# fernandezdaniel/MOBOCMF

Measured on AMD Instinct MI355X. Metric: ELBO steps/sec (MFDGP d=8 M=512 N=8192 S=8), higher is better.
Workload: dtype f64

## Files before the change

include/mobocmf_hip.h:

```cpp
#ifndef MOBOCMF_HIP_H
#define MOBOCMF_HIP_H

#include <stddef.h>
#include <stdint.h>

#ifdef __cplusplus
extern "C" {
#endif

typedef void* mobocmf_stream_t;

#define MOBOCMF_MAX_D 32
#define MOBOCMF_MAX_XDIV 48

enum {
    MOBOCMF_OK = 0,
    MOBOCMF_BAD_ARG = 1,
    MOBOCMF_WORKSPACE_TOO_SMALL = 2,
    MOBOCMF_HIP_ERROR = 3,
    MOBOCMF_NOT_PD = 4,
    MOBOCMF_BAD_ARCH = 5
};

typedef struct mobocmf_tuning {
    uint32_t struct_size;
    int32_t small_gemm_max;
    int32_t small_panel_max;
    int32_t tile_rows;
    int32_t pair_mode;
    int32_t mid_gemm_max;
    int32_t mid_gemm_waves;
    int32_t syrk_workgroups;
    int32_t sparse_backward;
    int32_t potrf_cols;
} mobocmf_tuning;
int mobocmf_tuning_init(mobocmf_tuning* t);

typedef struct {
    int32_t kind;
    int32_t d;
    int32_t M;
    int32_t xdiv;
    int64_t Np;
    int32_t branch;
    int32_t want_dx;
    double jitter;
    double min_var;
    int32_t phase;
    int32_t reserved;
// ... 363 lines not shown
```

mobocmf_amd/_lib.py:

```python
import ctypes
import os

_HERE = os.path.dirname(os.path.abspath(__file__))
LIB_PATH = os.environ.get("MOBOCMF_HIP_LIB") or os.path.join(_HERE, "csrc", "libmobocmf_hip.so")

OK, BAD_ARG, WORKSPACE_TOO_SMALL, HIP_ERROR, NOT_PD, BAD_ARCH = range(6)
_ERR = {1: "MOBOCMF_BAD_ARG", 2: "MOBOCMF_WORKSPACE_TOO_SMALL", 3: "MOBOCMF_HIP_ERROR", 4: "MOBOCMF_NOT_PD",
        5: "MOBOCMF_BAD_ARCH"}


class Tuning(ctypes.Structure):
    _fields_ = [("struct_size", ctypes.c_uint32), ("small_gemm_max", ctypes.c_int32), ("small_panel_max", ctypes.c_int32),
                ("tile_rows", ctypes.c_int32), ("pair_mode", ctypes.c_int32), ("mid_gemm_max", ctypes.c_int32),
                ("mid_gemm_waves", ctypes.c_int32), ("syrk_workgroups", ctypes.c_int32), ("sparse_backward", ctypes.c_int32),
                ("potrf_cols", ctypes.c_int32)]
    KNOBS = tuple(n for n, _ in _fields_[1:])

    def copy(self):
        t = Tuning()
        ctypes.memmove(ctypes.byref(t), ctypes.byref(self), ctypes.sizeof(Tuning))
        return t


PROBE_EVENTS = 11


class LayerDesc(ctypes.Structure):
    _fields_ = [("kind", ctypes.c_int32), ("d", ctypes.c_int32), ("M", ctypes.c_int32), ("xdiv", ctypes.c_int32),
                ("Np", ctypes.c_int64), ("branch", ctypes.c_int32), ("want_dx", ctypes.c_int32),
                ("jitter", ctypes.c_double), ("min_var", ctypes.c_double), ("phase", ctypes.c_int32),
                ("reserved", ctypes.c_int32), ("tuning", ctypes.POINTER(Tuning)), ("probe_events", ctypes.c_void_p)]
# ... 213 lines not shown
```

mobocmf_amd/csrc/api.hip:

```cpp
#include "common.h"

int launch_gram_fwd(const GramArgs& g, hipStream_t s);
int launch_gram_bwd(const GramArgs& g, bool want_dx, hipStream_t s);
void gram_grid(const GramArgs& g, dim3* grid);
int launch_sum_partials(const double* part, int64_t P, int64_t stride, double* out, int64_t len, double scale,
                        int accumulate, hipStream_t s);
int launch_potrf(double* A, int64_t ld, int Mp, int M, double* Dinv, double* Ld, int32_t* info, hipStream_t s);
int launch_trtri(const double* L, int64_t ld, int Mp, const double* Dinv, double* Linv, double* T, double* ws,
                 int64_t ws_elems, hipStream_t s);
int launch_pad_tril(const double* src, int64_t lds, int M, double* dst, int Mp, hipStream_t s);
int launch_pad_vec(const double* src, int64_t n, double* dst, int64_t np, hipStream_t s);
int launch_transpose(const double* in, int64_t ldi, double* out, int64_t ldo, int64_t rows, int64_t cols, hipStream_t s);
int launch_gemv_rows(const double* Mat, int64_t ld, const double* vec, double* out, int rows, int64_t cols, double scale,
                     int accumulate, hipStream_t s);
int launch_kl(const double* L, const double* LSp, const double* U, const double* a, int M, int Mp, double* kl,
              double* part, hipStream_t s);
int launch_moments_finish(const double* qpart, const double* mupart, const double* rpart, int nrb, int64_t Np, int64_t N,
                          const double* knn, int branch, double min_var, double* q, double* r, double* varraw,
                          double* mean, double* var, int32_t* zero_word, hipStream_t s);
int launch_moments_bwd_prep(const double* g_mean, const double* g_var, const double* knn, const double* q,
                            const double* varraw, int branch, double min_var, int64_t N, int64_t Np, double* gmu,
                            double* gv, double* gv2, double* cgv, int32_t* nclamped, int zeroed, int32_t* blkact, hipStream_t s);
int launch_reduce_slabs_sym(const double* slabs, int64_t slab_stride, int nslab, int nslab_diag, double* out, int Mp, const int32_t* flag,
                            const double* fallback, hipStream_t s);
// ... 29 lines not shown
int launch_gemv_rows_z(const double* Mat, int64_t ld, const double* vec, double* out, int rows, int64_t cols, double scale,
                       int accumulate, int nz, int64_t zs, hipStream_t s);
int launch_transpose_pad_z(const double* in, double* out, int Mp, const double* const* LS, const double* const* m, int M,
                           double* LSp, double* mp, int nz, int64_t zs, hipStream_t s);
int launch_transpose_gemv_z(const double* in, double* out, int Mp, const double* Mat, const double* vec, double* vout, int nz,
                            int64_t zs, hipStream_t s);
int launch_kl_z(const double* L, const double* LSp, const double* U, const double* a, int M, int Mp, double* const* kl,
                double* part, int nz, int64_t zs, hipStream_t s);
int launch_dutot_y_z(const double* G1, const double* G2, const double* Hc, const double* U, const double* da, const double* a,
                     const double* const* gkl, int Mp, double* dU, double* da_tot, double* Y, int nz, int64_t zs, hipStream_t s);
int launch_dl_from_t2_z(const double* T2, const double* L, const double* const* gkl, int M, int Mp, double* dL, int nz,
                        int64_t zs, hipStream_t s);
int launch_phi_z(const double* T3, int Mp, double* P, int nz, int64_t zs, hipStream_t s);
int launch_symmetrize_z(const double* S, int Mp, double* G, int nz, int64_t zs, hipStream_t s);

static const mobocmf_tuning kDefaultTuning = {(uint32_t)sizeof(mobocmf_tuning), 384, 512, 0, 0, 1024, 32, 0, 1, 0};
static thread_local const mobocmf_tuning* t_tuning = nullptr;
static thread_local void* const* t_probe = nullptr;
const mobocmf_tuning& tune() { return t_tuning ? *t_tuning : kDefaultTuning; }
bool tuning_ok(const mobocmf_tuning* t) {
    if (!t) return true;
    return t->struct_size == sizeof(mobocmf_tuning) && t->small_gemm_max >= 1 && t->small_gemm_max <= 512 &&
           t->small_panel_max >= 1 && t->small_panel_max <= 512 && (t->tile_rows == 0 || t->tile_rows == 64 || t->tile_rows == 128) &&
           t->pair_mode >= 0 && t->pair_mode <= 2 && t->mid_gemm_max >= 0 && t->mid_gemm_max <= 4096 &&
           (t->mid_gemm_waves == 4 || t->mid_gemm_waves == 8 || t->mid_gemm_waves == 32) &&
           (t->syrk_workgroups == 0 || (t->syrk_workgroups >= 16 && t->syrk_workgroups <= 4096)) &&
           (t->sparse_backward == 0 || t->sparse_backward == 1) && (t->potrf_cols == 0 || t->potrf_cols == 1 || t->potrf_cols == 4);
}
TuneScope::TuneScope(const mobocmf_tuning* t, void* const* probe) : prev_t(t_tuning), prev_p(t_probe) {
    t_tuning = t;
    t_probe = probe;
}
TuneScope::~TuneScope() {
    t_tuning = prev_t;
    t_probe = prev_p;
}
void probe_at(int i, hipStream_t s) {
    if (t_probe && i < MOBOCMF_PROBE_EVENTS && t_probe[i]) (void)hipEventRecord((hipEvent_t)t_probe[i], s);
}
static void set_pairing(GemmArgs& g) { g.pair_mode = tune().pair_mode; }
static int panel_tile_rows(int, int64_t) { return tune().tile_rows; }

#define TRY(x)              \
    do {                    \
// ... 1051 lines not shown
```

mobocmf_amd/csrc/common.h:

```cpp
#pragma once
#include <hip/hip_runtime.h>
#include <stdint.h>

#include "../../include/mobocmf_hip.h"

#define TILE 128
#define NB 64

static inline int64_t round_up(int64_t v, int64_t m) { return (v + m - 1) / m * m; }

#define HIP_TRY(expr)                                   \
    do {                                                \
        hipError_t _e = (expr);                         \
        if (_e != hipSuccess) return MOBOCMF_HIP_ERROR; \
    } while (0)

const mobocmf_tuning& tune();
bool tuning_ok(const mobocmf_tuning* t);
void probe_at(int i, hipStream_t s);
struct TuneScope {
    const mobocmf_tuning* prev_t;
    void* const* prev_p;
    explicit TuneScope(const mobocmf_tuning* t, void* const* probe = nullptr);
    ~TuneScope();
    TuneScope(const TuneScope&) = delete;
    TuneScope& operator=(const TuneScope&) = delete;
};

enum { TRI_NONE = 0, TRI_LOWER_A = 1, TRI_UPPER_A = 2, TRI_LOWER_B = 4, TRI_UPPER_B = 8 };
enum { EPI_STORE = 0, EPI_COLSTATS = 1, EPI_DA = 2 };

struct GemmArgs {
    const double* A;
    const double* B;
    double* C;
    int64_t lda, ldb, ldc;
    int Mr;
// ... 115 lines not shown
```

mobocmf_amd/csrc/elementwise.hip:

```cpp
#include "common.h"

#define LOG_2PI 1.8378770664093454835606594728112

__device__ __forceinline__ double wave_sum(double v) {
    v += __shfl_xor(v, 1);
    v += __shfl_xor(v, 2);
    v += __shfl_xor(v, 4);
    v += __shfl_xor(v, 8);
    v += __shfl_xor(v, 16);
    v += __shfl_xor(v, 32);
    return v;
}

__device__ __forceinline__ double block_sum(double v, double* sh) {
    v = wave_sum(v);
    const int lane = threadIdx.x & 63, wave = threadIdx.x >> 6;
    __syncthreads();
    if (lane == 0) sh[wave] = v;
    __syncthreads();
    double t = 0.0;
    if (threadIdx.x == 0)
        for (int w = 0; w < (int)(blockDim.x >> 6); ++w) t += sh[w];
    return t;
}
// ... 300 lines not shown
        if (threadIdx.x < 2) {
            const int64_t blk = (int64_t)blockIdx.x * 2 + threadIdx.x;
            if (blk * 128 < Np) blkact[blk] = any_w[2 * threadIdx.x] | any_w[2 * threadIdx.x + 1];
        }
    }
}
int launch_moments_bwd_prep(const double* g_mean, const double* g_var, const double* knn, const double* q,
                            const double* varraw, int branch, double min_var, int64_t N, int64_t Np, double* gmu,
                            double* gv, double* gv2, double* cgv, int32_t* nclamped, int zeroed, int32_t* blkact, hipStream_t s) {
    if (!zeroed && launch_zero32(nclamped, 1, s)) return MOBOCMF_HIP_ERROR;
    hipLaunchKernelGGL(moments_bwd_prep_kernel, GRID1(Np), 0, s, g_mean, g_var, knn, q, varraw, branch, min_var, N, Np,
                       gmu, gv, gv2, cgv, nclamped, blkact);
    return CHECK_LAUNCH();
}

__device__ __forceinline__ double slab_sum(const double* p, int64_t slab_stride, int ns) {
    double v = 0.0;
    int z = 0;
    for (; z + 8 <= ns; z += 8) {
        double t[8];
#pragma unroll
        for (int b = 0; b < 8; ++b) t[b] = p[(z + b) * slab_stride];
#pragma unroll
        for (int b = 0; b < 8; ++b) v += t[b];
    }
    for (; z < ns; ++z) v += p[z * slab_stride];
    return v;
}

__global__ void reduce_slabs_sym_kernel(const double* slabs, int64_t slab_stride, int nslab, int nslab_diag, double* out,
                                        int Mp, const int32_t* flag, const double* fallback) {
    int64_t idx = (int64_t)blockIdx.x * blockDim.x + threadIdx.x;
    if (idx >= (int64_t)Mp * Mp) return;
    int i = (int)(idx / Mp), j = (int)(idx % Mp);
    if (flag && *flag == 0) {
        out[idx] = fallback[idx];
        return;
    }
    if (j / TILE > i / TILE) return;
    const double* p = j > i ? slabs + (int64_t)j * Mp + i : slabs + (int64_t)i * Mp + j;
    const int ns = (i / TILE == j / TILE) ? nslab_diag : nslab;
    const double v = slab_sum(p, slab_stride, ns);
    out[idx] = v;
    if (j / TILE < i / TILE) out[(int64_t)j * Mp + i] = v;
}
__global__ void reduce_slabs_sym2_kernel(const double* slabs, const double* slabs2, int64_t slab_stride, int nslab,
                                         int nslab_diag, double* out, double* out2, int Mp, const int32_t* flag) {
    int64_t idx = (int64_t)blockIdx.x * blockDim.x + threadIdx.x;
    if (idx >= (int64_t)Mp * Mp) return;
    int i = (int)(idx / Mp), j = (int)(idx % Mp);
    if (j / TILE > i / TILE) return;
    const int64_t off = j > i ? (int64_t)j * Mp + i : (int64_t)i * Mp + j;
    const int ns = (i / TILE == j / TILE) ? nslab_diag : nslab;
    const double v = slab_sum(slabs + off, slab_stride, ns);
    double v2 = v;
    if (*flag != 0) v2 = slab_sum(slabs2 + off, slab_stride, ns);
    out[idx] = v;
    out2[idx] = v2;
    if (j / TILE < i / TILE) { out[(int64_t)j * Mp + i] = v; out2[(int64_t)j * Mp + i] = v2; }
}
int launch_reduce_slabs_sym2(const double* slabs, const double* slabs2, int64_t slab_stride, int nslab, int nslab_diag,
                             double* out, double* out2, int Mp, const int32_t* flag, hipStream_t s) {
    hipLaunchKernelGGL(reduce_slabs_sym2_kernel, GRID1((int64_t)Mp * Mp), 0, s, slabs, slabs2, slab_stride, nslab, nslab_diag,
                       out, out2, Mp, flag);
    return CHECK_LAUNCH();
}
int launch_reduce_slabs_sym(const double* slabs, int64_t slab_stride, int nslab, int nslab_diag, double* out, int Mp,
                            const int32_t* flag, const double* fallback, hipStream_t s) {
    hipLaunchKernelGGL(reduce_slabs_sym_kernel, GRID1((int64_t)Mp * Mp), 0, s, slabs, slab_stride, nslab, nslab_diag, out, Mp,
                       flag, fallback);
    return CHECK_LAUNCH();
}

__global__ void dutot_y_kernel(const double* G1, const double* G2, const double* Hc, const double* U, const double* da,
                               const double* a, ScalZ gklz, int Mp, double* dU, double* da_tot, double* Y, int64_t zs) {
    __shared__ double tl[32][33];
    const double* gkl = gklz.p[blockIdx.z];
    const double g = gkl ? gkl[0] : 0.0;
    const int64_t zo = blockIdx.z * zs;
    G1 += zo; G2 += zo; Hc += zo; U += zo; da += zo; a += zo; dU += zo; da_tot += zo; Y += zo;
    const int nt = Mp / 32, ti = blockIdx.x / nt, tj = blockIdx.x % nt;
    const int tx = threadIdx.x & 31, ty = threadIdx.x >> 5;
    if (tj <= ti) {
#pragma unroll
        for (int r = ty; r < 32; r += 8) tl[r][tx] = G1[(int64_t)(tj * 32 + r) * Mp + ti * 32 + tx];
// ... 1115 lines not shown
```

mobocmf_amd/csrc/gemm_f64.hip:

```cpp
#include "common.h"
#include <type_traits>
#include <atomic>

typedef double v4f64 __attribute__((ext_vector_type(4)));
typedef double v2f64 __attribute__((ext_vector_type(2)));

#define BM 128
#define BN 128
#define BK 16
#define KL_MAX 1024
#define TILE_ELEMS (BM * BK)

#ifndef GEMM_MI
#define GEMM_MI 16
#endif
#if GEMM_MI == 16
#define IMG_SWZ(row) ((((row) >> 1) & 1) | ((((row) >> 3) & 1) << 2))
#else
#define IMG_SWZ(row) ((((row) >> 1) & 1) << 2)
#endif


template <int CTRL>
__device__ __forceinline__ double dpp_mov(double v) {
// ... 51 lines not shown
#define STEP_STAMPS_DECL unsigned long long sst[10] = {0, 0, 0, 0, 0, 0, 0, 0, 0, 0};
#define STEP_STAMP(i) do { if (sbase >= 0) sst[sbase + (i)] = __builtin_amdgcn_s_memrealtime(); } while (0)
#define STEP_STAMPS_FLUSH                                                                                   \
    do {                                                                                                    \
        if (g_stamp_buf && threadIdx.x == 0)                                                                \
            for (int q = 0; q < 10; ++q) g_stamp_buf[(int64_t)blockIdx.x * 32 + 16 + q] = sst[q];           \
    } while (0)
#else
#define STAMP(i)
#define STAMP_ID()
#define STEP_STAMPS_DECL
#define STEP_STAMP(i)
#define STEP_STAMPS_FLUSH
#endif

template <bool B_T, bool TRI, int EPI, int RM>
__global__ __launch_bounds__(256, RM == 64 ? 3 : 2) void gemm_f64_kernel(GemmArgs g, int nrb, int64_t ncb, int splitk, int pair) {
    static_assert(RM == 128 || (RM == 64 && !B_T), "tile heights: 128, or 64 for the A B form");
    constexpr int MT = RM / 32;
    constexpr int A_ELEMS = RM * BK;
    constexpr int STAGE_ELEMS = A_ELEMS + TILE_ELEMS;
    __shared__ __attribute__((aligned(16))) double lds[2 * STAGE_ELEMS];
    __shared__ int kl[B_T ? KL_MAX : 1];
    __shared__ int kl_wsum[4];
    if (g.skip_if_zero && *g.skip_if_zero == 0) return;
    STAMP(0);
    STAMP_ID();
    int64_t id = blockIdx.x;
    if (g.dual_flag) {
        const int64_t half = (int64_t)(gridDim.x >> 1);
        if (id >= half) {
            if (*g.dual_flag == 0) return;
            id -= half;
            g.bscale = g.bscale2;
            g.C = g.C2;
        }
    }
    int rb, z = 0, sk_eff = splitk;
    int64_t cb;
    if (g.batched) {
        z = blockIdx.z;
        cb = id / nrb;
        rb = nrb - 1 - (int)(id % nrb);
    } else if (splitk > 1 && g.lower_out && g.splitk_diag > 0) {
        const int64_t nF = (int64_t)nrb * (nrb - 1) / 2, nblkF = nF * splitk;
        const bool diag = id >= nblkF;
        const int64_t id2 = diag ? id - nblkF : id, nT = diag ? nrb : nF;
        sk_eff = diag ? g.splitk_diag : splitk;
        int64_t t;
        if ((sk_eff & 7) == 0 && (nblkF & 7) == 0) {
            const int64_t xcd = id2 & 7, seq = id2 >> 3;
            t = seq % nT;
            z = (int)((seq / nT) * 8 + xcd);
        } else {
            t = id2 % nT;
            z = (int)(id2 / nT);
        }
        if (diag) {
            rb = (int)t;
            cb = t;
        } else {
            int r = 1;
            while ((int64_t)r * (r + 1) / 2 <= t) ++r;
            rb = r;
            cb = t - (int64_t)r * (r - 1) / 2;
        }
    } else if (splitk > 1) {
        const int64_t ntile = g.lower_out ? (int64_t)nrb * (nrb + 1) / 2 : (int64_t)nrb * ncb;
        int64_t t;
        if ((splitk & 7) == 0) {
            const int64_t xcd = id & 7, seq = id >> 3;
            t = seq % ntile;
            z = (int)((seq / ntile) * 8 + xcd);
        } else {
            t = id % ntile;
            z = (int)(id / ntile);
        }
        if (g.lower_out) {
            int r = 0;
            while ((int64_t)(r + 1) * (r + 2) / 2 <= t) ++r;
            rb = r;
            cb = t - (int64_t)r * (r + 1) / 2;
        } else {
            cb = t / nrb;
            rb = (int)(t % nrb);
        }
    } else {
        const int nslot = pair ? (nrb + 1) / 2 : nrb;
        int sl;
        if ((ncb & 7) == 0) {
            int64_t xcd = id & 7, slot = id >> 3;
            cb = (slot / nslot) * 8 + xcd;
            sl = (int)(slot % nslot);
        } else {
            cb = id / nslot;
            sl = (int)(id % nslot);
        }
        rb = pair ? sl : nrb - 1 - sl;
    }
    if (g.lower_out && cb > rb) return;

    const double* A = g.A;
    const double* B = g.B;
    double* C = g.C;
    if (g.batched) {
        const int zl = g.zlayers > 1 ? z % g.zlayers : 0;
        const int zb = g.zlayers > 1 ? z / g.zlayers : z;
        A += zb * g.strideA + zl * g.zsA;
        B += zb * g.strideB + zl * g.zsB;
        C += zb * g.strideC + zl * g.zsC;
    }
    if (!g.batched && splitk > 1) {
        C += z * g.slab_stride;
        if (g.zlayers > 1) {
            A += blockIdx.z * g.zsA;
            B += blockIdx.z * g.zsB;
            C += blockIdx.z * g.zsC;
        }
    }
    const int nparts = (pair && rb != nrb - 1 - rb) ? 2 : 1;
    const int rb_first = rb;

    const int tid = threadIdx.x;
    const int lane = tid & 63;
    const int wave = __builtin_amdgcn_readfirstlane(tid >> 6);
    const int wr = wave >> 1, wc = wave & 1;
    const int li = lane & 15, lk = lane >> 4;

    if constexpr (!B_T) {
        if (g.colact && g.colact[cb] == 0) {
            if (EPI == EPI_DA && g.rowdot_part) {
                for (int part = 0; part < nparts; ++part) {
                    const int rbp = part == 0 ? rb_first : nrb - 1 - rb_first;
                    for (int i = tid; i < 2 * RM; i += 256)
// ... 57 lines not shown
    if (g.tri & TRI_LOWER_B) {
        int64_t b = cb * BN;
        if (k0 < b) k0 = b;
    }
    if (g.tri & TRI_UPPER_B) {
        int64_t e = (cb + 1) * BN;
        if (k1 > e) k1 = e;
    }
    bool compact = false;
    int64_t ct0 = 0;
    int co0 = 0;
    if (!g.batched && splitk > 1) {
        bool sliced = false;
        if constexpr (B_T) {
            if (g.kact) {
                const int nb = (int)(g.Kd / 128), run = (nb + 255) / 256;
                const int rb0 = tid * run < nb ? tid * run : nb, rb1 = rb0 + run < nb ? rb0 + run : nb;
                int cnt = 0;
                for (int b = rb0; b < rb1; ++b) cnt += g.kact[b] != 0 ? 1 : 0;
                int inc = cnt;
#pragma unroll
                for (int off = 1; off < 64; off <<= 1) {
                    const int v = __shfl_up(inc, off);
                    if (lane >= off) inc += v;
                }
                if (lane == 63) kl_wsum[wave] = inc;
                __syncthreads();
                int ord = inc - cnt;
                for (int w = 0; w < wave; ++w) ord += kl_wsum[w];
                const int64_t nkt = (int64_t)(kl_wsum[0] + kl_wsum[1] + kl_wsum[2] + kl_wsum[3]) * (128 / BK);
                const int64_t per = (nkt + sk_eff - 1) / sk_eff;
                const int64_t tb = z * per < nkt ? z * per : nkt, te = tb + per < nkt ? tb + per : nkt;
                ct0 = tb;
                co0 = (int)(tb / (128 / BK));
                const int co1 = te > tb ? (int)((te - 1) / (128 / BK)) : co0 - 1;
                for (int b = rb0; b < rb1; ++b)
                    if (g.kact[b] != 0) {
                        if (ord >= co0 && ord <= co1 && ord - co0 < KL_MAX) kl[ord - co0] = b;
                        ++ord;
                    }
                __syncthreads();
                compact = true;
                sliced = true;
                k0 = 0;
                k1 = (te - tb) * BK;
            }
        }
        if (!sliced) {
            int64_t nkt = k1 > k0 ? (k1 - k0) / BK : 0;
            int64_t per = (nkt + sk_eff - 1) / sk_eff;
            int64_t b = k0 + z * per * BK, e = b + per * BK;
            k0 = b < k1 ? b : k1;
            k1 = e < k1 ? e : k1;
        }
    }
    const double* Ag = Ag0 + (int64_t)rb * RM * g.lda;

    v4f64 acc[MT][4];
#pragma unroll
    for (int i = 0; i < MT; ++i)
#pragma unroll
        for (int j = 0; j < 4; ++j) acc[i][j] = (v4f64){0.0, 0.0, 0.0, 0.0};

    const int64_t nk = (k1 > k0) ? (k1 - k0) / BK : 0;
#define KSTEP(KT) (rev ? nk - 1 - (KT) : (KT))
    auto koff = [&](int64_t kt) -> int64_t {
        if (B_T && compact) {
            const int64_t t = ct0 + kt;
            return (int64_t)kl[(int)(t / (128 / BK)) - co0] * 128 + (t % (128 / BK)) * BK;
        }
        return k0 + KSTEP(kt) * BK;
    };
#define KOFF(KT) koff(KT)
    if (nk > 0) stage(Ag, KOFF(0), 0);

    asm volatile("s_waitcnt vmcnt(0)" ::: "memory");
    __syncthreads();
    STAMP(1 + 4 * part);
    v4f64 w_nxt = (v4f64){1.0, 1.0, 1.0, 1.0};
    if (B_T && g.bscale && nk > 0) w_nxt = *(const v4f64*)(g.bscale + KOFF(0) + 4 * lk);
#if GEMM_MI == 16
    v2f64 fa[MT][2];
    double fb[4][4];
#define LOAD_A16(MT_)                                                                                       \
    fa[MT_][0] = *(const v2f64*)(As + a_base + (MT_) * 32 * BK + colP0);                                    \
// ... 359 lines not shown
    }
#define ST_PLAIN(v, p) (*(p) = (v))
#define ST_STREAM(v, p) __builtin_nontemporal_store((v), (p))
    if (g.accumulate) { STORE_TILE(ST_PLAIN, ST_PLAIN, 1) }
    else if (g.stream_out) { STORE_TILE(ST_STREAM, ST_STREAM, 0) }
    else { STORE_TILE(ST_PLAIN, ST_PLAIN, 0) }
#undef STORE_TILE
    if (part == 0) STAMP(13);

#undef COLOFF
    STAMP(9 + part);
  }
  STEP_STAMPS_FLUSH;
}

static bool small_panel_ok(const GemmArgs& g, bool B_T, int splitk);
template <int EPI> static int launch_small_panel(const GemmArgs& g, hipStream_t s);
static bool small_gemm_ok(const GemmArgs& g, bool B_T);
static int launch_small_gemm(const GemmArgs& g, bool B_T, hipStream_t s);

static int tile_rows(const GemmArgs& g, bool B_T, int splitk) {
    if (B_T || splitk > 1 || g.batched || g.lower_out || g.zlayers > 1) return BM;
    if (g.rm == 64 || g.rm == BM) return g.rm;
    if (!(g.tri & (TRI_LOWER_A | TRI_UPPER_A))) return BM;
    const int64_t pairs128 = (int64_t)((g.Mr / BM + 1) / 2) * (g.Nc / BN);
    return pairs128 >= 512 ? BM : 64;
}

int launch_gemm(const GemmArgs& g0, bool B_T, int splitk, hipStream_t s) {
    GemmArgs g = g0;
    if (g.Mr % BM || g.Nc % 16 || g.Kd % BK) return MOBOCMF_BAD_ARG;
    if (B_T || g.batched || splitk > 1) g.colact = nullptr;
    if (g.kact) {
        const int sk_min = (g.lower_out && g.splitk_diag > 0 && g.splitk_diag < splitk) ? g.splitk_diag : splitk;
        const int64_t nb = g.Kd / 128;
        if (!B_T || g.batched || splitk <= 1 || g.zlayers > 1 || g.Kd % 128 || (g.tri & (TRI_LOWER_B | TRI_UPPER_B)) ||
            (nb + sk_min - 1) / sk_min + 2 > KL_MAX)
            g.kact = nullptr;
    }
    if (!B_T && ((g.ldc & 1) || ((uintptr_t)g.C & 15))) return MOBOCMF_BAD_ARG;
    if (small_panel_ok(g, B_T, splitk)) {
// ... 29 lines not shown
    const bool tri = (g.tri & (TRI_LOWER_A | TRI_UPPER_A)) != 0 || g.epi == EPI_STORE;
#ifdef GEMM_LDS_PAD64
    const size_t dyn64 = GEMM_LDS_PAD64;
#define LAUNCH(BT, TR, EP, RM_)                                                                                         \
    do {                                                                                                                \
        const size_t dyn = (RM_) == 64 ? dyn64 : 0;                                                                     \
        if (dyn) (void)hipFuncSetAttribute((const void*)gemm_f64_kernel<BT, TR, EP, RM_>,                               \
                                           hipFuncAttributeMaxDynamicSharedMemorySize, (int)dyn);                       \
        hipLaunchKernelGGL((gemm_f64_kernel<BT, TR, EP, RM_>), grid, dim3(256), dyn, s, g, nrb, ncb, splitk, pair);      \
    } while (0)
#else
#define LAUNCH(BT, TR, EP, RM_) hipLaunchKernelGGL((gemm_f64_kernel<BT, TR, EP, RM_>), grid, dim3(256), 0, s, g, nrb, ncb, splitk, pair)
#endif
    if (B_T) {
        if (g.epi != EPI_STORE) return MOBOCMF_BAD_ARG;
        LAUNCH(true, false, EPI_STORE, 128);
    } else if (rm == 64) {
        if (g.epi == EPI_COLSTATS) LAUNCH(false, true, EPI_COLSTATS, 64);
        else if (g.epi == EPI_DA) LAUNCH(false, true, EPI_DA, 64);
        else LAUNCH(false, true, EPI_STORE, 64);
    } else if (tri) {
        if (g.epi == EPI_COLSTATS) LAUNCH(false, true, EPI_COLSTATS, 128);
        else if (g.epi == EPI_DA) LAUNCH(false, true, EPI_DA, 128);
        else LAUNCH(false, true, EPI_STORE, 128);
    } else {
        if (g.epi == EPI_COLSTATS) LAUNCH(false, false, EPI_COLSTATS, 128);
        else if (g.epi == EPI_DA) LAUNCH(false, false, EPI_DA, 128);
        else LAUNCH(false, false, EPI_STORE, 128);
    }
#undef LAUNCH
    return hipGetLastError() == hipSuccess ? MOBOCMF_OK : MOBOCMF_HIP_ERROR;
// ... 736 lines not shown
```

mobocmf_amd/functional.py:

```python
import contextlib
import ctypes
import os
import threading

import torch

from . import _lib
from ._lib import LayerDesc

JITTER = 1e-6
MIN_VARIANCE = 1e-10

_scratch = {}


def _stream():
    return ctypes.c_void_p(torch.cuda.current_stream().cuda_stream)


def _ptr(t):
    return ctypes.c_void_p(0 if t is None else t.data_ptr())


def _prep(t):
# ... 76 lines not shown
    if _TUNING_DEFAULT is None:
        t = _lib.Tuning()
        _lib.check(_lib.load().mobocmf_tuning_init(ctypes.byref(t)), "mobocmf_tuning_init")
        _TUNING_DEFAULT = t
    return _TUNING_DEFAULT


def current_tuning():
    t = getattr(_tuning_tls, "override", None)
    return (t if t is not None else _default_tuning()).copy()


def _set_default(**kw):
    t = _default_tuning()
    for k, v in kw.items():
        assert k in _lib.Tuning.KNOBS, k
        setattr(t, k, int(v))


@contextlib.contextmanager
def tuning(**kw):
    prev = getattr(_tuning_tls, "override", None)
    t = current_tuning()
    for k, v in kw.items():
        if k not in _lib.Tuning.KNOBS:
            raise TypeError("unknown tuning knob %r" % k)
        setattr(t, k, int(v))
    _tuning_tls.override = t
    try:
        yield t
    finally:
        _tuning_tls.override = prev


_probe_tls = threading.local()


@contextlib.contextmanager
def probe_events(table, layer=None):
    prev = getattr(_probe_tls, "cur", None)
# ... 1275 lines not shown
    _set_default(mid_gemm_max=n)


def set_mid_gemm_waves(n=32):
    if int(n) not in (4, 8, 32):
        raise _lib.MobocmfError("set_mid_gemm_waves: 4 | 8 | 32")
    _set_default(mid_gemm_waves=n)


def set_syrk_workgroups(n=0):
    if int(n) != 0 and not 16 <= int(n) <= 4096:
        raise _lib.MobocmfError("set_syrk_workgroups: 0 | 16..4096")
    _set_default(syrk_workgroups=n)


def set_sparse_backward(on=True):
    _set_default(sparse_backward=1 if on else 0)


_block_act_tls = threading.local()


def set_block_activity(act=None):
    if act is not None:
        assert act.dtype == torch.int32 and act.is_cuda and act.is_contiguous()
    _block_act_tls.act = act


def set_tile_rows(rows=0, pair_mode=0):
    if int(rows) not in (0, 64, 128) or not 0 <= int(pair_mode) <= 2:
# ... 559 lines not shown
```

Before: 1069.

## Add 8-wave SYRK kernel option and vectorize symmetric slab reduction

Adds a new 512-thread, 8-wave split-K SYRK kernel for symmetric lower-output GEMMs. It is selected only through a new syrk_waves tuning knob, which defaults to off, and the tuning struct gains a backward-compatible field. Separately, the symmetric slab-reduction kernels now load two doubles at a time and use larger unrolled batches. Each thread covers its own lower-triangle entries and mirrors them, replacing the old tile-granular mapping. These changes aim to cut the memory-bound reduction cost and, when the knob is set, the SYRK launch cost, at the price of extra code paths and alignment checks.

```diff
diff --git a/include/mobocmf_hip.h b/include/mobocmf_hip.h
--- a/include/mobocmf_hip.h
+++ b/include/mobocmf_hip.h
@@ -33,6 +33,7 @@
     int32_t syrk_workgroups;
     int32_t sparse_backward;
     int32_t potrf_cols;
+    int32_t syrk_waves;
 } mobocmf_tuning;
 int mobocmf_tuning_init(mobocmf_tuning* t);
 
diff --git a/mobocmf_amd/_lib.py b/mobocmf_amd/_lib.py
--- a/mobocmf_amd/_lib.py
+++ b/mobocmf_amd/_lib.py
@@ -13,8 +13,9 @@
     _fields_ = [("struct_size", ctypes.c_uint32), ("small_gemm_max", ctypes.c_int32), ("small_panel_max", ctypes.c_int32),
                 ("tile_rows", ctypes.c_int32), ("pair_mode", ctypes.c_int32), ("mid_gemm_max", ctypes.c_int32),
                 ("mid_gemm_waves", ctypes.c_int32), ("syrk_workgroups", ctypes.c_int32), ("sparse_backward", ctypes.c_int32),
-                ("potrf_cols", ctypes.c_int32)]
-    KNOBS = tuple(n for n, _ in _fields_[1:])
+                ("potrf_cols", ctypes.c_int32), ("syrk_waves", ctypes.c_int32)]
+    KNOBS = tuple(n for n, _ in _fields_[1:10])
+    ALL_KNOBS = tuple(n for n, _ in _fields_[1:])
 
     def copy(self):
         t = Tuning()
diff --git a/mobocmf_amd/csrc/api.hip b/mobocmf_amd/csrc/api.hip
--- a/mobocmf_amd/csrc/api.hip
+++ b/mobocmf_amd/csrc/api.hip
@@ -1,3 +1,5 @@
+#include <string.h>
+#include <stddef.h>
 #include "common.h"
 
 int launch_gram_fwd(const GramArgs& g, hipStream_t s);
@@ -67,20 +69,34 @@
 int launch_phi_z(const double* T3, int Mp, double* P, int nz, int64_t zs, hipStream_t s);
 int launch_symmetrize_z(const double* S, int Mp, double* G, int nz, int64_t zs, hipStream_t s);
 
-static const mobocmf_tuning kDefaultTuning = {(uint32_t)sizeof(mobocmf_tuning), 384, 512, 0, 0, 1024, 32, 0, 1, 0};
+static const mobocmf_tuning kDefaultTuning = {(uint32_t)sizeof(mobocmf_tuning), 384, 512, 0, 0, 1024, 32, 0, 1, 0, 0};
+static const uint32_t kTuningSizeV1 = (uint32_t)offsetof(mobocmf_tuning, syrk_waves);
 static thread_local const mobocmf_tuning* t_tuning = nullptr;
 static thread_local void* const* t_probe = nullptr;
 const mobocmf_tuning& tune() { return t_tuning ? *t_tuning : kDefaultTuning; }
 bool tuning_ok(const mobocmf_tuning* t) {
     if (!t) return true;
+    if (t->struct_size == kTuningSizeV1) {
+        mobocmf_tuning full = kDefaultTuning;
+        memcpy(&full, t, kTuningSizeV1);
+        full.struct_size = (uint32_t)sizeof(mobocmf_tuning);
+        return tuning_ok(&full);
+    }
     return t->struct_size == sizeof(mobocmf_tuning) && t->small_gemm_max >= 1 && t->small_gemm_max <= 512 &&
            t->small_panel_max >= 1 && t->small_panel_max <= 512 && (t->tile_rows == 0 || t->tile_rows == 64 || t->tile_rows == 128) &&
            t->pair_mode >= 0 && t->pair_mode <= 2 && t->mid_gemm_max >= 0 && t->mid_gemm_max <= 4096 &&
            (t->mid_gemm_waves == 4 || t->mid_gemm_waves == 8 || t->mid_gemm_waves == 32) &&
            (t->syrk_workgroups == 0 || (t->syrk_workgroups >= 16 && t->syrk_workgroups <= 4096)) &&
-           (t->sparse_backward == 0 || t->sparse_backward == 1) && (t->potrf_cols == 0 || t->potrf_cols == 1 || t->potrf_cols == 4);
+           (t->sparse_backward == 0 || t->sparse_backward == 1) && (t->potrf_cols == 0 || t->potrf_cols == 1 || t->potrf_cols == 4) &&
+           (t->syrk_waves == 0 || t->syrk_waves == 4 || t->syrk_waves == 8);
 }
 TuneScope::TuneScope(const mobocmf_tuning* t, void* const* probe) : prev_t(t_tuning), prev_p(t_probe) {
+    if (t && t->struct_size == kTuningSizeV1) {
+        widened = kDefaultTuning;
+        memcpy(&widened, t, kTuningSizeV1);
+        widened.struct_size = (uint32_t)sizeof(mobocmf_tuning);
+        t = &widened;
+    }
     t_tuning = t;
     t_probe = probe;
 }
diff --git a/mobocmf_amd/csrc/common.h b/mobocmf_amd/csrc/common.h
--- a/mobocmf_amd/csrc/common.h
+++ b/mobocmf_amd/csrc/common.h
@@ -21,6 +21,7 @@
 struct TuneScope {
     const mobocmf_tuning* prev_t;
     void* const* prev_p;
+    mobocmf_tuning widened;
     explicit TuneScope(const mobocmf_tuning* t, void* const* probe = nullptr);
     ~TuneScope();
     TuneScope(const TuneScope&) = delete;
diff --git a/mobocmf_amd/csrc/elementwise.hip b/mobocmf_amd/csrc/elementwise.hip
--- a/mobocmf_amd/csrc/elementwise.hip
+++ b/mobocmf_amd/csrc/elementwise.hip
@@ -338,61 +338,121 @@
     return CHECK_LAUNCH();
 }
 
-__device__ __forceinline__ double slab_sum(const double* p, int64_t slab_stride, int ns) {
-    double v = 0.0;
+typedef double slab_v2 __attribute__((ext_vector_type(2)));
+template <int BATCH, bool FULL, typename T, typename LD>
+__device__ __forceinline__ void slab_batch(T& v, const LD& ld, int z, int ns) {
+    T t[BATCH];
+#pragma unroll
+    for (int b = 0; b < BATCH; ++b) t[b] = ld(FULL || z + b < ns ? z + b : ns - 1);
+#pragma unroll
+    for (int b = 0; b < BATCH; ++b)
+        if (FULL || z + b < ns) v += t[b];
+}
+template <typename T, typename LD>
+__device__ __forceinline__ T slab_sum(const LD& ld, int ns) {
+    T v = {};
     int z = 0;
-    for (; z + 8 <= ns; z += 8) {
-        double t[8];
-#pragma unroll
-        for (int b = 0; b < 8; ++b) t[b] = p[(z + b) * slab_stride];
-#pragma unroll
-        for (int b = 0; b < 8; ++b) v += t[b];
-    }
-    for (; z < ns; ++z) v += p[z * slab_stride];
+    for (; z + 32 <= ns; z += 32) slab_batch<32, true>(v, ld, z, ns);
+    const int rem = ns - z;
+    if (rem > 16) slab_batch<32, false>(v, ld, z, ns);
+    else if (rem > 8) slab_batch<16, false>(v, ld, z, ns);
+    else if (rem > 0) slab_batch<8, false>(v, ld, z, ns);
     return v;
 }
-
-__global__ void reduce_slabs_sym_kernel(const double* slabs, int64_t slab_stride, int nslab, int nslab_diag, double* out,
-                                        int Mp, const int32_t* flag, const double* fallback) {
-    int64_t idx = (int64_t)blockIdx.x * blockDim.x + threadIdx.x;
+__device__ __forceinline__ slab_v2 slab_sum_v2(const double* p0, int64_t slab_stride, int ns) {
+    const slab_v2* p = (const slab_v2*)p0;
+    const int64_t st = slab_stride >> 1;
+    return slab_sum<slab_v2>([=](int z) { return p[z * st]; }, ns);
+}
+__device__ __forceinline__ double slab_sum_one(const double* p, int64_t slab_stride, int ns) {
+    return slab_sum<double>([=](int z) { return p[z * slab_stride]; }, ns);
+}
+
+template <int W>
+__global__ __launch_bounds__(256) void reduce_slabs_sym_kernel(const double* slabs, int64_t slab_stride, int nslab, int nslab_diag,
+                                                               double* out, int Mp, const int32_t* flag, const double* fallback) {
+    const int64_t idx = ((int64_t)blockIdx.x * blockDim.x + threadIdx.x) * W;
     if (idx >= (int64_t)Mp * Mp) return;
-    int i = (int)(idx / Mp), j = (int)(idx % Mp);
+    const int i = (int)(idx / Mp), j = (int)(idx % Mp);
     if (flag && *flag == 0) {
-        out[idx] = fallback[idx];
+        if (W == 2) *(slab_v2*)(out + idx) = *(const slab_v2*)(fallback + idx);
+        else out[idx] = fallback[idx];
         return;
     }
-    if (j / TILE > i / TILE) return;
-    const double* p = j > i ? slabs + (int64_t)j * Mp + i : slabs + (int64_t)i * Mp + j;
+    if (j > i) return;
     const int ns = (i / TILE == j / TILE) ? nslab_diag : nslab;
-    const double v = slab_sum(p, slab_stride, ns);
-    out[idx] = v;
-    if (j / TILE < i / TILE) out[(int64_t)j * Mp + i] = v;
-}
-__global__ void reduce_slabs_sym2_kernel(const double* slabs, const double* slabs2, int64_t slab_stride, int nslab,
-                                         int nslab_diag, double* out, double* out2, int Mp, const int32_t* flag) {
-    int64_t idx = (int64_t)blockIdx.x * blockDim.x + threadIdx.x;
+    if (W == 2) {
+        const slab_v2 v = slab_sum_v2(slabs + idx, slab_stride, ns);
+        if (j == i) {
+            out[idx] = v[0];
+        } else {
+            *(slab_v2*)(out + idx) = v;
+            out[(int64_t)j * Mp + i] = v[0];
+            if (j + 1 < i) out[(int64_t)(j + 1) * Mp + i] = v[1];
+        }
+    } else {
+        const double v = slab_sum_one(slabs + idx, slab_stride, ns);
+        out[idx] = v;
+        if (j < i) out[(int64_t)j * Mp + i] = v;
+    }
+}
+template <int W>
+__global__ __launch_bounds__(256) void reduce_slabs_sym2_kernel(const double* slabs, const double* slabs2, int64_t slab_stride,
+                                                                int nslab, int nslab_diag, double* out, double* out2, int Mp,
+                                                                const int32_t* flag) {
+    const int64_t idx = ((int64_t)blockIdx.x * blockDim.x + threadIdx.x) * W;
     if (idx >= (int64_t)Mp * Mp) return;
-    int i = (int)(idx / Mp), j = (int)(idx % Mp);
-    if (j / TILE > i / TILE) return;
-    const int64_t off = j > i ? (int64_t)j * Mp + i : (int64_t)i * Mp + j;
+    const int i = (int)(idx / Mp), j = (int)(idx % Mp);
+    if (j > i) return;
     const int ns = (i / TILE == j / TILE) ? nslab_diag : nslab;
-    const double v = slab_sum(slabs + off, slab_stride, ns);
-    double v2 = v;
-    if (*flag != 0) v2 = slab_sum(slabs2 + off, slab_stride, ns);
-    out[idx] = v;
-    out2[idx] = v2;
-    if (j / TILE < i / TILE) { out[(int64_t)j * Mp + i] = v; out2[(int64_t)j * Mp + i] = v2; }
+    const bool twin = *flag != 0;
+    if (W == 2) {
+        const slab_v2 v = slab_sum_v2(slabs + idx, slab_stride, ns);
+        slab_v2 v2 = v;
+        if (twin) v2 = slab_sum_v2(slabs2 + idx, slab_stride, ns);
+        if (j == i) {
+            out[idx] = v[0];
+            out2[idx] = v2[0];
+        } else {
+            *(slab_v2*)(out + idx) = v;
+            *(slab_v2*)(out2 + idx) = v2;
+            out[(int64_t)j * Mp + i] = v[0];
+            out2[(int64_t)j * Mp + i] = v2[0];
+            if (j + 1 < i) {
+                out[(int64_t)(j + 1) * Mp + i] = v[1];
+                out2[(int64_t)(j + 1) * Mp + i] = v2[1];
+            }
+        }
+    } else {
+        const double v = slab_sum_one(slabs + idx, slab_stride, ns);
+        double v2 = v;
+        if (twin) v2 = slab_sum_one(slabs2 + idx, slab_stride, ns);
+        out[idx] = v;
+        out2[idx] = v2;
+        if (j < i) { out[(int64_t)j * Mp + i] = v; out2[(int64_t)j * Mp + i] = v2; }
+    }
+}
+static bool aligned16(const void* a, const void* b, const void* c, const void* d) {
+    return ((((uintptr_t)a) | ((uintptr_t)b) | ((uintptr_t)c) | ((uintptr_t)d)) & 15) == 0;
 }
 int launch_reduce_slabs_sym2(const double* slabs, const double* slabs2, int64_t slab_stride, int nslab, int nslab_diag,
                              double* out, double* out2, int Mp, const int32_t* flag, hipStream_t s) {
-    hipLaunchKernelGGL(reduce_slabs_sym2_kernel, GRID1((int64_t)Mp * Mp), 0, s, slabs, slabs2, slab_stride, nslab, nslab_diag,
-                       out, out2, Mp, flag);
+    if (aligned16(slabs, slabs2, out, out2) && !(slab_stride & 1))
+        hipLaunchKernelGGL(reduce_slabs_sym2_kernel<2>, GRID1((int64_t)Mp * Mp / 2), 0, s, slabs, slabs2, slab_stride, nslab,
+                           nslab_diag, out, out2, Mp, flag);
+    else
+        hipLaunchKernelGGL(reduce_slabs_sym2_kernel<1>, GRID1((int64_t)Mp * Mp), 0, s, slabs, slabs2, slab_stride, nslab,
+                           nslab_diag, out, out2, Mp, flag);
     return CHECK_LAUNCH();
 }
 int launch_reduce_slabs_sym(const double* slabs, int64_t slab_stride, int nslab, int nslab_diag, double* out, int Mp,
                             const int32_t* flag, const double* fallback, hipStream_t s) {
-    hipLaunchKernelGGL(reduce_slabs_sym_kernel, GRID1((int64_t)Mp * Mp), 0, s, slabs, slab_stride, nslab, nslab_diag, out, Mp,
-                       flag, fallback);
+    if (aligned16(slabs, out, fallback, nullptr) && !(slab_stride & 1))
+        hipLaunchKernelGGL(reduce_slabs_sym_kernel<2>, GRID1((int64_t)Mp * Mp / 2), 0, s, slabs, slab_stride, nslab, nslab_diag,
+                           out, Mp, flag, fallback);
+    else
+        hipLaunchKernelGGL(reduce_slabs_sym_kernel<1>, GRID1((int64_t)Mp * Mp), 0, s, slabs, slab_stride, nslab, nslab_diag, out,
+                           Mp, flag, fallback);
     return CHECK_LAUNCH();
 }
 
diff --git a/mobocmf_amd/csrc/gemm_f64.hip b/mobocmf_amd/csrc/gemm_f64.hip
--- a/mobocmf_amd/csrc/gemm_f64.hip
+++ b/mobocmf_amd/csrc/gemm_f64.hip
@@ -89,23 +89,20 @@
 #define STEP_STAMPS_FLUSH
 #endif
 
-template <bool B_T, bool TRI, int EPI, int RM>
-__global__ __launch_bounds__(256, RM == 64 ? 3 : 2) void gemm_f64_kernel(GemmArgs g, int nrb, int64_t ncb, int splitk, int pair) {
-    static_assert(RM == 128 || (RM == 64 && !B_T), "tile heights: 128, or 64 for the A B form");
-    constexpr int MT = RM / 32;
-    constexpr int A_ELEMS = RM * BK;
-    constexpr int STAGE_ELEMS = A_ELEMS + TILE_ELEMS;
-    __shared__ __attribute__((aligned(16))) double lds[2 * STAGE_ELEMS];
-    __shared__ int kl[B_T ? KL_MAX : 1];
-    __shared__ int kl_wsum[4];
-    if (g.skip_if_zero && *g.skip_if_zero == 0) return;
-    STAMP(0);
-    STAMP_ID();
+struct TileId {
+    int rb;
+    int64_t cb;
+    int z;
+    int sk_eff;
+};
+
+__device__ __forceinline__ bool gemm_tile_of_block(GemmArgs& g, int nrb, int64_t ncb, int splitk, int pair, TileId& t) {
+    if (g.skip_if_zero && *g.skip_if_zero == 0) return false;
     int64_t id = blockIdx.x;
     if (g.dual_flag) {
         const int64_t half = (int64_t)(gridDim.x >> 1);
         if (id >= half) {
-            if (*g.dual_flag == 0) return;
+            if (*g.dual_flag == 0) return false;
             id -= half;
             g.bscale = g.bscale2;
             g.C = g.C2;
@@ -122,43 +119,43 @@
         const bool diag = id >= nblkF;
         const int64_t id2 = diag ? id - nblkF : id, nT = diag ? nrb : nF;
         sk_eff = diag ? g.splitk_diag : splitk;
-        int64_t t;
+        int64_t tl;
         if ((sk_eff & 7) == 0 && (nblkF & 7) == 0) {
             const int64_t xcd = id2 & 7, seq = id2 >> 3;
-            t = seq % nT;
+            tl = seq % nT;
             z = (int)((seq / nT) * 8 + xcd);
         } else {
-            t = id2 % nT;
+            tl = id2 % nT;
             z = (int)(id2 / nT);
         }
         if (diag) {
-            rb = (int)t;
-            cb = t;
+            rb = (int)tl;
+            cb = tl;
         } else {
             int r = 1;
-            while ((int64_t)r * (r + 1) / 2 <= t) ++r;
+            while ((int64_t)r * (r + 1) / 2 <= tl) ++r;
             rb = r;
-            cb = t - (int64_t)r * (r - 1) / 2;
+            cb = tl - (int64_t)r * (r - 1) / 2;
         }
     } else if (splitk > 1) {
         const int64_t ntile = g.lower_out ? (int64_t)nrb * (nrb + 1) / 2 : (int64_t)nrb * ncb;
-        int64_t t;
+        int64_t tl;
         if ((splitk & 7) == 0) {
             const int64_t xcd = id & 7, seq = id >> 3;
-            t = seq % ntile;
+            tl = seq % ntile;
             z = (int)((seq / ntile) * 8 + xcd);
         } else {
-            t = id % ntile;
+            tl = id % ntile;
             z = (int)(id / ntile);
         }
         if (g.lower_out) {
             int r = 0;
-            while ((int64_t)(r + 1) * (r + 2) / 2 <= t) ++r;
+            while ((int64_t)(r + 1) * (r + 2) / 2 <= tl) ++r;
             rb = r;
-            cb = t - (int64_t)r * (r + 1) / 2;
+            cb = tl - (int64_t)r * (r + 1) / 2;
         } else {
-            cb = t / nrb;
-            rb = (int)(t % nrb);
+            cb = tl / nrb;
+            rb = (int)(tl % nrb);
         }
     } else {
         const int nslot = pair ? (nrb + 1) / 2 : nrb;
@@ -173,11 +170,19 @@
         }
         rb = pair ? sl : nrb - 1 - sl;
     }
-    if (g.lower_out && cb > rb) return;
-
-    const double* A = g.A;
-    const double* B = g.B;
-    double* C = g.C;
+    if (g.lower_out && cb > rb) return false;
+    t.rb = rb;
+    t.cb = cb;
+    t.z = z;
+    t.sk_eff = sk_eff;
+    return true;
+}
+
+__device__ __forceinline__ void gemm_operand_bases(const GemmArgs& g, int z, int splitk, const double*& A, const double*& B,
+                                                   double*& C) {
+    A = g.A;
+    B = g.B;
+    C = g.C;
     if (g.batched) {
         const int zl = g.zlayers > 1 ? z % g.zlayers : 0;
         const int zb = g.zlayers > 1 ? z / g.zlayers : z;
@@ -193,6 +198,73 @@
             C += blockIdx.z * g.zsC;
         }
     }
+}
+
+template <int NT>
+__device__ __forceinline__ int64_t kact_slice(const GemmArgs& g, int z, int sk_eff, int* kl, int* kl_wsum, int tid, int lane,
+                                              int wave, int64_t& ct0, int& co0) {
+    const int nb = (int)(g.Kd / 128), run = (nb + NT - 1) / NT;
+    const int rb0 = tid * run < nb ? tid * run : nb, rb1 = rb0 + run < nb ? rb0 + run : nb;
+    int cnt = 0;
+    for (int b = rb0; b < rb1; ++b) cnt += g.kact[b] != 0 ? 1 : 0;
+    int inc = cnt;
+#pragma unroll
+    for (int off = 1; off < 64; off <<= 1) {
+        const int v = __shfl_up(inc, off);
+        if (lane >= off) inc += v;
+    }
+    if (lane == 63) kl_wsum[wave] = inc;
+    __syncthreads();
+    int ord = inc - cnt, nact = 0;
+    for (int w = 0; w < wave; ++w) ord += kl_wsum[w];
+#pragma unroll
+    for (int w = 0; w < NT / 64; ++w) nact += kl_wsum[w];
+    const int64_t nkt = (int64_t)nact * (128 / BK);
+    const int64_t per = (nkt + sk_eff - 1) / sk_eff;
+    const int64_t tb = z * per < nkt ? z * per : nkt, te = tb + per < nkt ? tb + per : nkt;
+    ct0 = tb;
+    co0 = (int)(tb / (128 / BK));
+    const int co1 = te > tb ? (int)((te - 1) / (128 / BK)) : co0 - 1;
+    for (int b = rb0; b < rb1; ++b)
+        if (g.kact[b] != 0) {
+            if (ord >= co0 && ord <= co1 && ord - co0 < KL_MAX) kl[ord - co0] = b;
+            ++ord;
+        }
+    __syncthreads();
+    return te - tb;
+}
+__device__ __forceinline__ int64_t kact_koff(const int* kl, int64_t ct0, int co0, int64_t kt) {
+    const int64_t t = ct0 + kt;
+    return (int64_t)kl[(int)(t / (128 / BK)) - co0] * 128 + (t % (128 / BK)) * BK;
+}
+__device__ __forceinline__ void k_slice(int64_t& k0, int64_t& k1, int z, int sk_eff) {
+    const int64_t nkt = k1 > k0 ? (k1 - k0) / BK : 0;
+    const int64_t per = (nkt + sk_eff - 1) / sk_eff;
+    const int64_t b = k0 + z * per * BK, e = b + per * BK;
+    k0 = b < k1 ? b : k1;
+    k1 = e < k1 ? e : k1;
+}
+
+template <bool B_T, bool TRI, int EPI, int RM>
+__global__ __launch_bounds__(256, RM == 64 ? 3 : 2) void gemm_f64_kernel(GemmArgs g, int nrb, int64_t ncb, int splitk, int pair) {
+    static_assert(RM == 128 || (RM == 64 && !B_T), "tile heights: 128, or 64 for the A B form");
+    constexpr int MT = RM / 32;
+    constexpr int A_ELEMS = RM * BK;
+    constexpr int STAGE_ELEMS = A_ELEMS + TILE_ELEMS;
+    __shared__ __attribute__((aligned(16))) double lds[2 * STAGE_ELEMS];
+    __shared__ int kl[B_T ? KL_MAX : 1];
+    __shared__ int kl_wsum[4];
+    TileId tile;
+    if (!gemm_tile_of_block(g, nrb, ncb, splitk, pair, tile)) return;
+    STAMP(0);
+    STAMP_ID();
+    int rb = tile.rb;
+    const int z = tile.z, sk_eff = tile.sk_eff;
+    const int64_t cb = tile.cb;
+
+    const double *A, *B;
+    double* C;
+    gemm_operand_bases(g, z, splitk, A, B, C);
     const int nparts = (pair && rb != nrb - 1 - rb) ? 2 : 1;
     const int rb_first = rb;
 
@@ -280,45 +352,14 @@
         bool sliced = false;
         if constexpr (B_T) {
             if (g.kact) {
-                const int nb = (int)(g.Kd / 128), run = (nb + 255) / 256;
-                const int rb0 = tid * run < nb ? tid * run : nb, rb1 = rb0 + run < nb ? rb0 + run : nb;
-                int cnt = 0;
-                for (int b = rb0; b < rb1; ++b) cnt += g.kact[b] != 0 ? 1 : 0;
-                int inc = cnt;
-#pragma unroll
-                for (int off = 1; off < 64; off <<= 1) {
-                    const int v = __shfl_up(inc, off);
-                    if (lane >= off) inc += v;
-                }
-                if (lane == 63) kl_wsum[wave] = inc;
-                __syncthreads();
-                int ord = inc - cnt;
-                for (int w = 0; w < wave; ++w) ord += kl_wsum[w];
-                const int64_t nkt = (int64_t)(kl_wsum[0] + kl_wsum[1] + kl_wsum[2] + kl_wsum[3]) * (128 / BK);
-                const int64_t per = (nkt + sk_eff - 1) / sk_eff;
-                const int64_t tb = z * per < nkt ? z * per : nkt, te = tb + per < nkt ? tb + per : nkt;
-                ct0 = tb;
-                co0 = (int)(tb / (128 / BK));
-                const int co1 = te > tb ? (int)((te - 1) / (128 / BK)) : co0 - 1;
-                for (int b = rb0; b < rb1; ++b)
-                    if (g.kact[b] != 0) {
-                        if (ord >= co0 && ord <= co1 && ord - co0 < KL_MAX) kl[ord - co0] = b;
-                        ++ord;
-                    }
-                __syncthreads();
+                const int64_t nsteps = kact_slice<256>(g, z, sk_eff, kl, kl_wsum, tid, lane, wave, ct0, co0);
                 compact = true;
                 sliced = true;
                 k0 = 0;
-                k1 = (te - tb) * BK;
+                k1 = nsteps * BK;
             }
         }
-        if (!sliced) {
-            int64_t nkt = k1 > k0 ? (k1 - k0) / BK : 0;
-            int64_t per = (nkt + sk_eff - 1) / sk_eff;
-            int64_t b = k0 + z * per * BK, e = b + per * BK;
-            k0 = b < k1 ? b : k1;
-            k1 = e < k1 ? e : k1;
-        }
+        if (!sliced) k_slice(k0, k1, z, sk_eff);
     }
     const double* Ag = Ag0 + (int64_t)rb * RM * g.lda;
 
@@ -331,10 +372,7 @@
     const int64_t nk = (k1 > k0) ? (k1 - k0) / BK : 0;
 #define KSTEP(KT) (rev ? nk - 1 - (KT) : (KT))
     auto koff = [&](int64_t kt) -> int64_t {
-        if (B_T && compact) {
-            const int64_t t = ct0 + kt;
-            return (int64_t)kl[(int)(t / (128 / BK)) - co0] * 128 + (t % (128 / BK)) * BK;
-        }
+        if (B_T && compact) return kact_koff(kl, ct0, co0, kt);
         return k0 + KSTEP(kt) * BK;
     };
 #define KOFF(KT) koff(KT)
@@ -724,6 +762,151 @@
   STEP_STAMPS_FLUSH;
 }
 
+#if GEMM_MI == 16
+#define W8_LE0 0xD5
+#define W8_LE1 0xF4
+#define W8_LT0 0x54
+#define W8_LT1 0xD0
+__global__ __launch_bounds__(512) void syrk_w8_kernel(GemmArgs g, int nrb, int64_t ncb, int splitk) {
+    constexpr int STAGE_ELEMS = 2 * TILE_ELEMS;
+    __shared__ __attribute__((aligned(16))) double lds[2 * STAGE_ELEMS];
+    __shared__ int kl[KL_MAX];
+    __shared__ int kl_wsum[8];
+    TileId tile;
+    if (!gemm_tile_of_block(g, nrb, ncb, splitk, 0, tile)) return;
+    const int rb = tile.rb, z = tile.z;
+    const int64_t cb = tile.cb;
+    const double *A, *B;
+    double* C;
+    gemm_operand_bases(g, z, splitk, A, B, C);
+
+    const int tid = threadIdx.x;
+    const int lane = tid & 63;
+    const int wave = __builtin_amdgcn_readfirstlane(tid >> 6);
+    const int wr = (wave >> 1) & 1, wc = wave & 1, h = wave >> 2;
+    const int li = lane & 15, lk = lane >> 4;
+
+    const int a_row = tid >> 3;
+    const int a_lchk = (tid & 7) ^ IMG_SWZ(a_row);
+    const double* Ag = A + ((int64_t)rb * BM + a_row) * g.lda + a_lchk * 2;
+    const double* Bg = B + (cb * BN + a_row) * g.ldb + a_lchk * 2;
+    auto stage = [&](int64_t k, int buf) {
+        double* As = lds + buf * STAGE_ELEMS;
+        double* Bs = As + TILE_ELEMS;
+#pragma unroll
+        for (int r = 0; r < 2; ++r) glds16(Ag + (int64_t)(64 * r) * g.lda + k, As + (r * 8 + wave) * 128);
+#pragma unroll
+        for (int r = 0; r < 2; ++r) glds16(Bg + (int64_t)(64 * r) * g.ldb + k, Bs + (r * 8 + wave) * 128);
+    };
+
+    int64_t k0 = 0, k1 = g.Kd, ct0 = 0;
+    int co0 = 0;
+    const bool compact = g.kact != nullptr;
+    if (compact) {
+        k1 = kact_slice<512>(g, z, tile.sk_eff, kl, kl_wsum, tid, lane, wave, ct0, co0) * BK;
+    } else {
+        k_slice(k0, k1, z, tile.sk_eff);
+    }
+    const int64_t nk = (k1 > k0) ? (k1 - k0) / BK : 0;
+    auto koff = [&](int64_t kt) -> int64_t { return compact ? kact_koff(kl, ct0, co0, kt) : k0 + kt * BK; };
+
+    const int swA = IMG_SWZ(li);
+    const int colP0 = ((2 * lk + 0) ^ swA) << 1, colP1 = ((2 * lk + 1) ^ swA) << 1;
+    const int a_base = (wr * 16 + li) * BK;
+    const int b_base0 = ((h ? 1 : 0) * 32 + wc * 16 + li) * BK;
+    const int b_base1 = ((h ? 2 : 3) * 32 + wc * 16 + li) * BK;
+
+    v4f64 acc[4][2];
+#pragma unroll
+    for (int i = 0; i < 4; ++i)
+#pragma unroll
+        for (int j = 0; j < 2; ++j) acc[i][j] = (v4f64){0.0, 0.0, 0.0, 0.0};
+
+    if (nk > 0) stage(koff(0), 0);
+    asm volatile("s_waitcnt vmcnt(0)" ::: "memory");
+    __syncthreads();
+    v4f64 w_nxt = (v4f64){1.0, 1.0, 1.0, 1.0};
+    if (g.bscale && nk > 0) w_nxt = *(const v4f64*)(g.bscale + koff(0) + 4 * lk);
+#ifdef SYRK_W8_PRIO
+    if (h) __builtin_amdgcn_s_setprio(1);
+#endif
+
+    v2f64 fa[4][2];
+    double fb[4][2];
+#define W8_ROW(MASK, MT_) ((((MASK) >> (2 * (MT_))) & 3) != 0)
+#define W8_COL(MASK, J) ((((MASK) >> (J)) & 0x55) != 0)
+#define W8_LOAD_A(MASK, MT_, CH)                                                                            \
+    if constexpr (W8_ROW(MASK, MT_)) fa[MT_][CH] = *(const v2f64*)(As + a_base + (MT_) * 32 * BK + ((CH) ? colP1 : colP0));
+#define W8_LOAD_B(MASK, J, CH)                                                                              \
+    if constexpr (W8_COL(MASK, J)) {                                                                        \
+        const v2f64 v = *(const v2f64*)(Bs + ((J) ? b_base1 : b_base0) + ((CH) ? colP1 : colP0));           \
+        fb[2 * (CH)][J] = v[0] * w4[2 * (CH)];                                                              \
+        fb[2 * (CH) + 1][J] = v[1] * w4[2 * (CH) + 1];                                                      \
+    }
+#define W8_MMA(MASK, Q, MT_, J)                                                                             \
+    if constexpr ((((MASK) >> (2 * (MT_) + (J))) & 1) != 0)                                                 \
+        acc[MT_][J] = __builtin_amdgcn_mfma_f64_16x16x4f64(fa[MT_][(Q) >> 1][(Q) & 1], fb[Q][J], acc[MT_][J], 0, 0, 0);
+#define W8_MMA_Q(MASK, Q)                                                                                   \
+    W8_MMA(MASK, Q, 0, 0) W8_MMA(MASK, Q, 0, 1) W8_MMA(MASK, Q, 1, 0) W8_MMA(MASK, Q, 1, 1)                 \
+    W8_MMA(MASK, Q, 2, 0) W8_MMA(MASK, Q, 2, 1) W8_MMA(MASK, Q, 3, 0) W8_MMA(MASK, Q, 3, 1)
+#define W8_LOOP(MASK)                                                                                       \
+    for (int64_t kt = 0; kt < nk; ++kt) {                                                                   \
+        const int buf = (int)(kt & 1);                                                                      \
+        const v4f64 w4 = w_nxt;                                                                             \
+        const double* As = lds + buf * STAGE_ELEMS;                                                         \
+        const double* Bs = As + TILE_ELEMS;                                                                 \
+        W8_LOAD_B(MASK, 0, 0) W8_LOAD_B(MASK, 1, 0)                                                         \
+        W8_LOAD_A(MASK, 0, 0) W8_LOAD_A(MASK, 1, 0) W8_LOAD_A(MASK, 2, 0) W8_LOAD_A(MASK, 3, 0)             \
+        if (kt + 1 < nk) {                                                                                  \
+                         \
+            const int64_t knext = koff(kt + 1);                                                             \
+            if (g.bscale) w_nxt = *(const v4f64*)(g.bscale + knext + 4 * lk);                               \
+            stage(knext, buf ^ 1);                                                                          \
+        }                                                                                                   \
+        W8_LOAD_B(MASK, 0, 1) W8_LOAD_B(MASK, 1, 1)                                                         \
+        W8_LOAD_A(MASK, 0, 1) W8_LOAD_A(MASK, 1, 1) W8_LOAD_A(MASK, 2, 1) W8_LOAD_A(MASK, 3, 1)             \
+        __builtin_amdgcn_sched_barrier(0);                                                                  \
+        W8_MMA_Q(MASK, 0) W8_MMA_Q(MASK, 1) W8_MMA_Q(MASK, 2) W8_MMA_Q(MASK, 3)                             \
+        __builtin_amdgcn_sched_barrier(0);                                                                  \
+            \
+        asm volatile("s_waitcnt vmcnt(0) lgkmcnt(0)" ::: "memory");                                         \
+        __syncthreads();                                                                                    \
+    }
+    if (g.sym_out && g.lower_out && rb == cb) {
+        const int role = __builtin_amdgcn_readfirstlane(((wr == 0 && wc == 1) ? 2 : 0) | h);
+        if (role == 0) { W8_LOOP(W8_LE0) }
+        else if (role == 1) { W8_LOOP(W8_LE1) }
+        else if (role == 2) { W8_LOOP(W8_LT0) }
+        else { W8_LOOP(W8_LT1) }
+    } else {
+        W8_LOOP(0xFF)
+    }
+#undef W8_LOOP
+#undef W8_MMA_Q
+#undef W8_MMA
+#undef W8_LOAD_B
+#undef W8_LOAD_A
+#undef W8_COL
+#undef W8_ROW
+#ifdef SYRK_W8_PRIO
+    if (h) __builtin_amdgcn_s_setprio(0);
+#endif
+
+    double* cp = C + ((int64_t)rb * BM + wr * 16 + lk) * g.ldc + cb * BN + wc * 16 + li;
+    const int c0 = (h ? 1 : 0) * 32, c1 = (h ? 2 : 3) * 32;
+#pragma unroll
+    for (int mt = 0; mt < 4; ++mt)
+#pragma unroll
+        for (int r = 0; r < 4; ++r) {
+            double* p = cp + (int64_t)(mt * 32 + 4 * r) * g.ldc;
+            p[c0] = g.alpha * acc[mt][0][r];
+            p[c1] = g.alpha * acc[mt][1][r];
+        }
+}
+#else
+__global__ void syrk_w8_kernel(GemmArgs, int, int64_t, int) {}
+#endif
+
 static bool small_panel_ok(const GemmArgs& g, bool B_T, int splitk);
 template <int EPI> static int launch_small_panel(const GemmArgs& g, hipStream_t s);
 static bool small_gemm_ok(const GemmArgs& g, bool B_T);
@@ -735,6 +918,19 @@
     if (!(g.tri & (TRI_LOWER_A | TRI_UPPER_A))) return BM;
     const int64_t pairs128 = (int64_t)((g.Mr / BM + 1) / 2) * (g.Nc / BN);
     return pairs128 >= 512 ? BM : 64;
+}
+
+static int syrk_waves(const GemmArgs& g, int splitk) {
+#if GEMM_MI == 16
+    const bool covered = splitk > 1 && !g.batched && g.sym_out && g.lower_out && g.tri == TRI_NONE && !g.accumulate &&
+                         !g.stream_out && g.zlayers <= 1;
+#else
+    const bool covered = false;
+#endif
+    if (!covered) return 4;
+    const int knob = tune().syrk_waves;
+    if (knob) return knob;
+    return 4;
 }
 
 int launch_gemm(const GemmArgs& g0, bool B_T, int splitk, hipStream_t s) {
@@ -794,7 +990,8 @@
 #endif
     if (B_T) {
         if (g.epi != EPI_STORE) return MOBOCMF_BAD_ARG;
-        LAUNCH(true, false, EPI_STORE, 128);
+        if (syrk_waves(g, splitk) == 8) hipLaunchKernelGGL(syrk_w8_kernel, grid, dim3(512), 0, s, g, nrb, ncb, splitk);
+        else LAUNCH(true, false, EPI_STORE, 128);
     } else if (rm == 64) {
         if (g.epi == EPI_COLSTATS) LAUNCH(false, true, EPI_COLSTATS, 64);
         else if (g.epi == EPI_DA) LAUNCH(false, true, EPI_DA, 64);
diff --git a/mobocmf_amd/functional.py b/mobocmf_amd/functional.py
--- a/mobocmf_amd/functional.py
+++ b/mobocmf_amd/functional.py
@@ -114,7 +114,7 @@
 def _set_default(**kw):
     t = _default_tuning()
     for k, v in kw.items():
-        assert k in _lib.Tuning.KNOBS, k
+        assert k in _lib.Tuning.ALL_KNOBS, k
         setattr(t, k, int(v))
 
 
@@ -123,7 +123,7 @@
     prev = getattr(_tuning_tls, "override", None)
     t = current_tuning()
     for k, v in kw.items():
-        if k not in _lib.Tuning.KNOBS:
+        if k not in _lib.Tuning.ALL_KNOBS:
             raise TypeError("unknown tuning knob %r" % k)
         setattr(t, k, int(v))
     _tuning_tls.override = t
@@ -1429,6 +1429,12 @@
     _set_default(syrk_workgroups=n)
 
 
+def set_syrk_waves(n=0):
+    if int(n) not in (0, 4, 8):
+        raise _lib.MobocmfError("set_syrk_waves: 0 | 4 | 8")
+    _set_default(syrk_waves=n)
+
+
 def set_sparse_backward(on=True):
     _set_default(sparse_backward=1 if on else 0)
 
```

New measurement: 1071 (median of 6 runs). Within noise of the previous version (+0.2%).
